# rrwick/Polypolish

Measured on AMD Instinct MI355X. Metric: assembly Mbp polished/sec at 200x coverage; bit-identical FASTA vs reference, higher is better.
Workload: dtype u8/u32 counts + f64 depth

## Files before the change

polypolish_amd/csrc/pp_k_emit.h:

```cpp
#pragma once

namespace pp {

__global__ __launch_bounds__(256) void k_sub_bases(const u8 *__restrict__ bases, const u64 *__restrict__ sub_off, u32 n_sub,
                                                   const u64 *__restrict__ src_start, u8 *__restrict__ out, u64 g_sub) {
    const u64 p0 = ((u64)blockIdx.x * blockDim.x + threadIdx.x) * 8ull;
    if (p0 >= g_sub) return;
    u32 lo = 0, hi = n_sub;
    while (hi - lo > 1) {
        const u32 mid = (lo + hi) >> 1;
        if (sub_off[mid] <= p0) lo = mid; else hi = mid;
    }
    if (p0 + 8 <= sub_off[lo + 1]) {
        u64 v;
        __builtin_memcpy(&v, bases + src_start[lo] + (p0 - sub_off[lo]), 8);
        __builtin_memcpy(out + p0, &v, 8);
        return;
    }
    for (u64 p = p0; p < min(p0 + 8, g_sub); p++) {
        while (p >= sub_off[lo + 1]) lo++;
        out[p] = bases[src_start[lo] + (p - sub_off[lo])];
    }
}

__device__ __forceinline__ u32 code_len(u8 c, u32 gp, const MultiEnt *multi, u32 n_multi) {
    if (c == 0) return 0;
    if (c < 0x80u) return 1;
    if (c != 0xFFu) return c & 0x7Fu;
    for (u32 i = 0; i < n_multi; i++)
        if (multi[i].pos == gp) return multi[i].eff;
    return 0;
}

#ifndef PP_EMIT_PPT
#define PP_EMIT_PPT 16
#endif
constexpr int EMIT_PPT = PP_EMIT_PPT;
static_assert(EMIT_PPT == 8 || EMIT_PPT == 16, "an 8- or 16-byte load of codes per thread");
constexpr int COMPACT_THREADS = TILE / EMIT_PPT;
constexpr u32 EMIT_FUSE_MAX = 4096;
template <u32 NTHREADS>
__device__ __forceinline__ u64 sum_part(const u32 *__restrict__ a, u32 n, u32 t) {
    u64 p = 0;
#pragma unroll 1
    for (u32 i0 = 4u * t; i0 < n; i0 += 16u * NTHREADS) {
        uint4 v[4];
#pragma unroll
        for (u32 j = 0; j < 4u; j++) {
            const u32 i = i0 + 4u * NTHREADS * j;
            v[j] = make_uint4(0u, 0u, 0u, 0u);
            if (i < n) v[j] = *(const uint4 *)(a + i);
        }
#pragma unroll
        for (u32 j = 0; j < 4u; j++) {
            const u32 i = i0 + 4u * NTHREADS * j;
            p += (u64)(i < n ? v[j].x : 0u) + (i + 1u < n ? v[j].y : 0u) + (i + 2u < n ? v[j].z : 0u) + (i + 3u < n ? v[j].w : 0u);
        }
    }
    return p;
}
template <u32 NTHREADS>
__device__ __forceinline__ u64 prefix_part(const u32 *__restrict__ win_coarse, const u32 *__restrict__ win_coarse2,
                                           const u32 *__restrict__ win_len, u32 w, u32 t) {
    static_assert(WIN_COARSE == 64 && WIN_COARSE2 == 64 * WIN_COARSE && NTHREADS >= 32, "two stretches of up to 64 elements: sixteen threads each");
    const u32 g = w / WIN_COARSE, g2 = w / WIN_COARSE2;
    const bool second = t >= 16u;
    const u32 *const a = second ? win_coarse + (u64)g2 * 64u : win_len + (u64)g * WIN_COARSE;
    const u32 n = second ? g - g2 * 64u : w - g * WIN_COARSE, i = 4u * (t & 15u);
    uint4 v = make_uint4(0u, 0u, 0u, 0u);
    if (t < 32u && i < n) v = *(const uint4 *)(a + i);
    u64 p = sum_part<NTHREADS>(win_coarse2, g2, t);
    if (t < 32u) p += (u64)(i < n ? v.x : 0u) + (i + 1u < n ? v.y : 0u) + (i + 2u < n ? v.z : 0u) + (i + 3u < n ? v.w : 0u);
    return p;
}

template <bool FUSED>
__device__ __forceinline__ void compact_window(u32 w, const u8 *__restrict__ code, u64 G,
                                               const u64 *__restrict__ win_out, const u32 *__restrict__ win_len, const u32 *__restrict__ win_coarse, const u32 *__restrict__ win_coarse2, u64 cap_out,
                                               const MultiEnt *__restrict__ multi,
                                               const u32 *__restrict__ counters,
                                               u8 *__restrict__ out, const u64 *__restrict__ status) {
    __shared__ u32 wsum[COMPACT_THREADS / 64];
    __shared__ u64 psum[COMPACT_THREADS / 64];
    const u32 t = threadIdx.x, lane = t & 63u, wave = t >> 6;
    const u64 p0 = (u64)w * TILE + (u64)EMIT_PPT * t;
    const bool whole = p0 + EMIT_PPT <= G;
    uint4 v = make_uint4(0u, 0u, 0u, 0u);
    if (whole) {
        if constexpr (EMIT_PPT == 16) v = *(const uint4 *)(code + p0);
        else { const uint2 h = *(const uint2 *)(code + p0); v.x = h.x; v.y = h.y; }
    }
    const u64 st = *status;
    u64 o0 = 0, o1 = 0, part = 0;
    if constexpr (FUSED) {
        o1 = win_len[w];
        part = prefix_part<COMPACT_THREADS>(win_coarse, win_coarse2, win_len, w, t);
    } else {
        o0 = win_out[w];
        o1 = win_out[w + 1];
    }
    const u32 n_multi = counters[MC_MULTI];
    asm volatile("" : "+v"(v.x), "+v"(v.y), "+v"(v.z), "+v"(v.w));
    if ((st != ~0ull) | (o1 == o0)) return;
    u8 c[EMIT_PPT];
    if (whole) {
        __builtin_memcpy(c, &v, EMIT_PPT);
    } else {
#pragma unroll
        for (int i = 0; i < EMIT_PPT; i++) c[i] = (p0 + i < G) ? code[p0 + i] : (u8)0;
    }
    u32 len[EMIT_PPT], s = 0;
    bool all_one = true;
#pragma unroll
    for (int i = 0; i < EMIT_PPT; i++) {
        len[i] = code_len(c[i], (u32)(p0 + i), multi, n_multi);
        s += len[i];
        all_one = all_one && c[i] != 0 && c[i] < 0x80u;
    }
    u32 inc = s;
    for (int o = 1; o < 64; o <<= 1) {
        u32 v2 = __shfl_up(inc, o, 64);
        if ((int)lane >= o) inc += v2;
    }
    if (lane == 63) wsum[wave] = inc;
    if constexpr (FUSED) {
        const u64 pw = wave_sum64(part);
        if (lane == 0) psum[wave] = pw;
    }
    __syncthreads();
    u32 base = 0;
    for (u32 i = 0; i < wave; i++) base += wsum[i];
    if constexpr (FUSED) {
        const u64 len_w = o1;
        o0 = 0;
        for (u32 i = 0; i < (u32)(COMPACT_THREADS / 64); i++) o0 += psum[i];
        if (o0 + len_w > cap_out) return;
    }
    u64 off = o0 + base + (inc - s);
    if (all_one) {
        __builtin_memcpy(out + off, c, EMIT_PPT);
    } else {
#pragma unroll
        for (int i = 0; i < EMIT_PPT; i++) {
            if (c[i] && c[i] < 0x80u) out[off] = c[i];
            off += len[i];
        }
    }
}

template <bool FUSED>
__device__ __forceinline__ void finalize_entries(u32 first_wave, u32 n_waves, const u8 *__restrict__ code, u64 G,
                                                 const u64 *__restrict__ win_out, u32 nwin,
                                                 const u32 *__restrict__ win_len, const u32 *__restrict__ win_coarse, const u32 *__restrict__ win_coarse2, u64 cap_out, u64 *__restrict__ total_out, u64 *status,
                                                 const MultiEnt *__restrict__ multi,
                                                 const u32 *__restrict__ counters,
                                                 const u8 *__restrict__ seq,
                                                 const u64 *__restrict__ contig_off, u32 n_contigs,
                                                 u8 *__restrict__ out, u64 *__restrict__ ctg_out) {
    const u32 n_multi = counters[MC_MULTI];
    const u32 lane = threadIdx.x & 63u;
    const u32 n_todo = n_multi + n_contigs + 1u;
    auto begin_of = [&](u32 w) -> u64 {
        if constexpr (FUSED) return wave_sum64(prefix_part<64>(win_coarse, win_coarse2, win_len, w, lane)); else return win_out[w];
    };
    for (u32 t = first_wave; t < n_todo; t += n_waves) {
        u64 gp;
        if (t < n_multi) gp = multi[t].pos; else gp = contig_off[t - n_multi];
        u64 off;
        if (gp >= G) {
            off = begin_of(nwin);
            if (FUSED && t == n_todo - 1u && lane == 0) {
                __hip_atomic_store(total_out, off, __ATOMIC_RELAXED, __HIP_MEMORY_SCOPE_AGENT);
                if (off > cap_out) report(status, off, DE_CAPACITY);
            }
        } else {
            const u32 w = (u32)(gp / TILE);
            u32 part = 0;
            bool emits;
            if constexpr (FUSED) emits = win_len[w] != 0u; else emits = win_out[w + 1] != win_out[w];
            if (emits)
                for (u64 q = (u64)w * TILE + lane; q < gp; q += 64) part += code_len(code[q], (u32)q, multi, n_multi);
            off = begin_of(w) + wave_sum(part);
        }
        if (t < n_multi) {
            if (lane == 0 && !(FUSED && off + multi[t].len > cap_out)) {
                const u8 *s = seq + multi[t].off;
                for (u32 b = 0; b < multi[t].len; b++)
                    if (s[b] != (u8)'-') out[off++] = s[b];
            }
        } else if (lane == 0) {
            __hip_atomic_store(&ctg_out[t - n_multi], off, __ATOMIC_RELAXED, __HIP_MEMORY_SCOPE_AGENT);
        }
    }
}

constexpr u32 EMIT_DONE_GROUP = 64, EMIT_DONE_STRIDE = 8;
__host__ __device__ constexpr u64 emit_done_words(u64 blocks) { return (1ull + (blocks + EMIT_DONE_GROUP - 1) / EMIT_DONE_GROUP) * EMIT_DONE_STRIDE; }
struct EmitTail {
    u64 *meta;
    u32 words;
    u32 reinit;
    u64 *host;
    u64 serial;
    u64 *done;
    u32 *zero_a, *zero_b, *zero_c, *zero_d;
    u32 n_zero;
    u32 *zero_e;
    u32 n_zero_e;
    u32 ordered;
};
__device__ __forceinline__ void emit_tail(const EmitTail &Z) {
    __shared__ u32 s_last;
    if (!Z.host) return;
#if defined(__HIP_DEVICE_COMPILE__) && !defined(__gfx950__) && !defined(__gfx942__)
#error "k_emit's last-workgroup hand-over relies on gfx942/gfx950 agent-scope store/load semantics"
#endif
    __builtin_amdgcn_s_waitcnt(0);
    __syncthreads();
    if (threadIdx.x == 0) {
        u64 *const mine = Z.done + (u64)EMIT_DONE_STRIDE * (1u + blockIdx.x / EMIT_DONE_GROUP);
        const u32 in_group = min(EMIT_DONE_GROUP, gridDim.x - blockIdx.x / EMIT_DONE_GROUP * EMIT_DONE_GROUP);
        bool last = false;
        if (__hip_atomic_fetch_add(mine, 1ull, __ATOMIC_RELAXED, __HIP_MEMORY_SCOPE_AGENT) == (u64)in_group - 1ull) {
            __hip_atomic_store(mine, 0ull, __ATOMIC_RELAXED, __HIP_MEMORY_SCOPE_AGENT);
            last = __hip_atomic_fetch_add(Z.done, 1ull, __ATOMIC_RELAXED, __HIP_MEMORY_SCOPE_AGENT) == (u64)((gridDim.x + EMIT_DONE_GROUP - 1u) / EMIT_DONE_GROUP) - 1ull;
            if (last) __hip_atomic_store(Z.done, 0ull, __ATOMIC_RELAXED, __HIP_MEMORY_SCOPE_AGENT);
        }
        s_last = last;
    }
    __syncthreads();
    if (!s_last) return;
    const u32 i0 = threadIdx.x;
    const u64 st = __hip_atomic_load(Z.meta + MW_STATUS, __ATOMIC_RELAXED, __HIP_MEMORY_SCOPE_AGENT);
    const u64 c01 = __hip_atomic_load(Z.meta + MW_COUNTERS, __ATOMIC_RELAXED, __HIP_MEMORY_SCOPE_AGENT);
    const u64 c23 = __hip_atomic_load(Z.meta + MW_COUNTERS + 1, __ATOMIC_RELAXED, __HIP_MEMORY_SCOPE_AGENT);
    u64 v = __hip_atomic_load(Z.meta + min(i0, Z.words - 1u), __ATOMIC_RELAXED, __HIP_MEMORY_SCOPE_AGENT);
    const bool flagged = (u32)c01 != 0u || (u32)c23 != 0u;
    const bool again = st == ~0ull && (Z.reinit == 2u || (Z.reinit == 1u && !flagged));
    __syncthreads();
    for (u32 i = i0; i < Z.words; i += blockDim.x) {
        if (i != i0) v = __hip_atomic_load(Z.meta + i, __ATOMIC_RELAXED, __HIP_MEMORY_SCOPE_AGENT);
        __hip_atomic_store(Z.host + i, v, __ATOMIC_RELAXED, __HIP_MEMORY_SCOPE_SYSTEM);
        if (again) Z.meta[i] = i == MW_STATUS ? ~0ull : 0ull;
    }
    if (!Z.ordered && threadIdx.x == 0) {
        __hip_atomic_store(Z.host + Z.words, again ? 1ull : 0ull, __ATOMIC_RELAXED, __HIP_MEMORY_SCOPE_SYSTEM);
        __hip_atomic_store(Z.host + Z.words + 1, Z.serial, __ATOMIC_RELAXED, __HIP_MEMORY_SCOPE_SYSTEM);
    }
    if (again) {
        for (u32 i = threadIdx.x; i < Z.n_zero_e; i += blockDim.x) Z.zero_e[i] = 0;
        if (Z.zero_a)
            for (u32 i = threadIdx.x; i < Z.n_zero; i += blockDim.x) { Z.zero_a[i] = 0; Z.zero_b[i] = 0; }
        if (Z.zero_c)
            for (u32 i = threadIdx.x; i < Z.n_zero; i += blockDim.x) { Z.zero_c[i] = 0; Z.zero_d[i] = 0; }
    }
    if (Z.ordered) {
        __builtin_amdgcn_s_waitcnt(0);
        __syncthreads();
        if (threadIdx.x == 0) {
            __hip_atomic_store(Z.host + Z.words, again ? 1ull : 0ull, __ATOMIC_RELAXED, __HIP_MEMORY_SCOPE_SYSTEM);
            __builtin_amdgcn_s_waitcnt(0);
            __hip_atomic_store(Z.host + Z.words + 1, Z.serial, __ATOMIC_RELAXED, __HIP_MEMORY_SCOPE_SYSTEM);
        }
    }
}

template <bool FUSED>
__global__ __launch_bounds__(COMPACT_THREADS) void k_emit(const u8 *__restrict__ code, u64 G, const u64 *__restrict__ win_out,
                                                          const u32 *__restrict__ win_len, const u32 *__restrict__ win_coarse, const u32 *__restrict__ win_coarse2, u64 cap_out, u64 *__restrict__ total_out,
                                                          u32 nwin, u32 n_work, const u32 *__restrict__ own_win,
                                                          const MultiEnt *__restrict__ multi,
                                                          const u32 *__restrict__ counters, const u8 *__restrict__ seq,
                                                          const u64 *__restrict__ contig_off, u32 n_contigs,
                                                          u8 *__restrict__ out, u64 *__restrict__ ctg_out,
                                                          u64 *__restrict__ status, EmitTail Z) {
    if (blockIdx.x < n_work) {
        u32 w = blockIdx.x;
        if (own_win) {
            const u32 nr = own_win[0];
            const u32 *first = own_win + 1, *before = own_win + 1 + nr;
            u32 lo = 0, hi = nr;
            while (hi - lo > 1) {
                const u32 mid = (lo + hi) >> 1;
                if (before[mid] <= w) lo = mid; else hi = mid;
            }
            w = first[lo] + (w - before[lo]);
        }
        compact_window<FUSED>(w, code, G, win_out, win_len, win_coarse, win_coarse2, cap_out, multi, counters, out, status);
    } else if (*status == ~0ull) {
        constexpr u32 WPB = COMPACT_THREADS / 64;
        finalize_entries<FUSED>((blockIdx.x - n_work) * WPB + (threadIdx.x >> 6), (gridDim.x - n_work) * WPB, code, G, win_out, nwin, win_len, win_coarse, win_coarse2, cap_out,
                         total_out, status, multi, counters, seq, contig_off, n_contigs, out, ctg_out);
    }
    emit_tail(Z);
}

}
```

Measured before the change: 18500.

## Parallelize finalize entries: vectorized prefix lengths, wave-wide sequence emit, finalize blocks first

Rewrites the finalize path of the emit kernel. Each lane now loads 16-byte chunks of the window's codes and counts emitted bytes with SWAR popcount, instead of a strided per-byte loop. The multi-entry sequence copy uses a ballot and popcount across the wave instead of a serial lane-0 loop, and the prefix computation loads speculatively without branches. Finalize blocks are reordered to the front of the grid so they start early instead of trailing the compaction blocks. This adds complexity and assumes TILE==2048.

```diff
diff --git a/polypolish_amd/csrc/pp_k_emit.h b/polypolish_amd/csrc/pp_k_emit.h
--- a/polypolish_amd/csrc/pp_k_emit.h
+++ b/polypolish_amd/csrc/pp_k_emit.h
@@ -71,6 +71,19 @@
     if (t < 32u && i < n) v = *(const uint4 *)(a + i);
     u64 p = sum_part<NTHREADS>(win_coarse2, g2, t);
     if (t < 32u) p += (u64)(i < n ? v.x : 0u) + (i + 1u < n ? v.y : 0u) + (i + 2u < n ? v.z : 0u) + (i + 3u < n ? v.w : 0u);
+    return p;
+}
+__device__ __forceinline__ u64 prefix_part_wave(const u32 *__restrict__ win_coarse, const u32 *__restrict__ win_coarse2,
+                                                const u32 *__restrict__ win_len, u32 w, u32 lane) {
+    const u32 g = w / WIN_COARSE, g2 = w / WIN_COARSE2;
+    const bool second = lane >= 16u;
+    const u32 *const a = second ? win_coarse + (u64)g2 * 64u : win_len + (u64)g * WIN_COARSE;
+    const u32 n = lane >= 32u ? 0u : (second ? g - g2 * 64u : w - g * WIN_COARSE), i = 4u * (lane & 15u);
+    const uint4 v = *(const uint4 *)(a + (i < n ? i : 0u));
+    const u32 c2 = win_coarse2[lane < g2 ? lane : 0u];
+    u64 p = (u64)(i < n ? v.x : 0u) + (i + 1u < n ? v.y : 0u) + (i + 2u < n ? v.z : 0u) + (i + 3u < n ? v.w : 0u) + (lane < g2 ? c2 : 0u);
+#pragma unroll 1
+    for (u32 j = lane + 64u; j < g2; j += 64u) p += win_coarse2[j];
     return p;
 }
 
@@ -148,6 +161,26 @@
     }
 }
 
+__device__ __forceinline__ u32 len_before(const uint4 &v, u64 q0, u64 end, const MultiEnt *multi, u32 n_multi) {
+    const u32 n = q0 < end ? (u32)min(end - q0, (u64)16) : 0u, x[4] = {v.x, v.y, v.z, v.w};
+    u32 s = 0;
+#pragma unroll
+    for (u32 j = 0; j < 4u; j++) {
+        const u32 nb = n > 4u * j ? min(n - 4u * j, 4u) : 0u;
+        const u32 y = nb == 4u ? x[j] : x[j] & ((1u << (8u * nb)) - 1u);
+        const u32 hi = y & 0x80808080u;
+        s += (u32)__popc((((y & 0x7F7F7F7Fu) + 0x7F7F7F7Fu) & 0x80808080u) & ~hi);
+        if (hi) {
+#pragma unroll 1
+            for (u32 b = 0; b < 4u; b++) {
+                const u32 c = (y >> (8u * b)) & 0xFFu;
+                if (c >= 0x80u) s += code_len((u8)c, (u32)(q0 + 4u * j + b), multi, n_multi);
+            }
+        }
+    }
+    return s;
+}
+
 template <bool FUSED>
 __device__ __forceinline__ void finalize_entries(u32 first_wave, u32 n_waves, const u8 *__restrict__ code, u64 G,
                                                  const u64 *__restrict__ win_out, u32 nwin,
@@ -161,11 +194,20 @@
     const u32 lane = threadIdx.x & 63u;
     const u32 n_todo = n_multi + n_contigs + 1u;
     auto begin_of = [&](u32 w) -> u64 {
-        if constexpr (FUSED) return wave_sum64(prefix_part<64>(win_coarse, win_coarse2, win_len, w, lane)); else return win_out[w];
+        if constexpr (FUSED) return wave_sum64(prefix_part_wave(win_coarse, win_coarse2, win_len, w, lane)); else return win_out[w];
     };
+    static_assert(TILE == 2048, "a window's codes: two 16-byte loads a lane");
     for (u32 t = first_wave; t < n_todo; t += n_waves) {
-        u64 gp;
-        if (t < n_multi) gp = multi[t].pos; else gp = contig_off[t - n_multi];
+        const bool winner = t < n_multi;
+        u64 gp, s_off = 0;
+        u32 s_len = 0;
+        if (winner) {
+            const MultiEnt m = multi[t];
+            gp = m.pos; s_off = m.off; s_len = m.len;
+        } else gp = contig_off[t - n_multi];
+        const bool has_bytes = winner && s_len != 0u;
+        u8 ch = (has_bytes ? seq + s_off : code)[has_bytes ? min(lane, s_len - 1u) : 0u];
+        if (lane >= s_len) ch = (u8)'-';
         u64 off;
         if (gp >= G) {
             off = begin_of(nwin);
@@ -175,18 +217,35 @@
             }
         } else {
             const u32 w = (u32)(gp / TILE);
+            const u64 q0 = (u64)w * TILE + 16u * lane, q1 = q0 + TILE / 2;
+            uint4 v0 = *(const uint4 *)(code + (q0 < gp ? q0 : 0)), v1 = *(const uint4 *)(code + (q1 < gp ? q1 : 0));
+            u64 o0, part64 = 0;
+            bool emits;
+            if constexpr (FUSED) {
+                emits = win_len[w] != 0u;
+                part64 = prefix_part_wave(win_coarse, win_coarse2, win_len, w, lane);
+            } else {
+                o0 = win_out[w];
+                emits = win_out[w + 1] != o0;
+            }
+            asm volatile("" : "+v"(v0.x), "+v"(v0.y), "+v"(v0.z), "+v"(v0.w), "+v"(v1.x), "+v"(v1.y), "+v"(v1.z), "+v"(v1.w), "+v"(part64));
+            if constexpr (FUSED) o0 = wave_sum64(part64);
             u32 part = 0;
-            bool emits;
-            if constexpr (FUSED) emits = win_len[w] != 0u; else emits = win_out[w + 1] != win_out[w];
             if (emits)
-                for (u64 q = (u64)w * TILE + lane; q < gp; q += 64) part += code_len(code[q], (u32)q, multi, n_multi);
-            off = begin_of(w) + wave_sum(part);
-        }
-        if (t < n_multi) {
-            if (lane == 0 && !(FUSED && off + multi[t].len > cap_out)) {
-                const u8 *s = seq + multi[t].off;
-                for (u32 b = 0; b < multi[t].len; b++)
-                    if (s[b] != (u8)'-') out[off++] = s[b];
+                part = len_before(v0, q0, gp, multi, n_multi) + len_before(v1, q1, gp, multi, n_multi);
+            off = o0 + wave_sum(part);
+        }
+        if (winner) {
+            if (!(FUSED && off + s_len > cap_out)) {
+                for (u32 b0 = 0;;) {
+                    const bool keep = ch != (u8)'-';
+                    const u64 kept = __ballot(keep);
+                    if (keep) out[off + (u32)__popcll(kept & ((1ull << lane) - 1ull))] = ch;
+                    off += (u32)__popcll(kept);
+                    b0 += 64u;
+                    if (b0 >= s_len) break;
+                    ch = b0 + lane < s_len ? seq[s_off + b0 + lane] : (u8)'-';
+                }
             }
         } else if (lane == 0) {
             __hip_atomic_store(&ctg_out[t - n_multi], off, __ATOMIC_RELAXED, __HIP_MEMORY_SCOPE_AGENT);
@@ -274,8 +333,9 @@
                                                           const u64 *__restrict__ contig_off, u32 n_contigs,
                                                           u8 *__restrict__ out, u64 *__restrict__ ctg_out,
                                                           u64 *__restrict__ status, EmitTail Z) {
-    if (blockIdx.x < n_work) {
-        u32 w = blockIdx.x;
+    const u32 n_fin = gridDim.x - n_work;
+    if (blockIdx.x >= n_fin) {
+        u32 w = blockIdx.x - n_fin;
         if (own_win) {
             const u32 nr = own_win[0];
             const u32 *first = own_win + 1, *before = own_win + 1 + nr;
@@ -289,7 +349,7 @@
         compact_window<FUSED>(w, code, G, win_out, win_len, win_coarse, win_coarse2, cap_out, multi, counters, out, status);
     } else if (*status == ~0ull) {
         constexpr u32 WPB = COMPACT_THREADS / 64;
-        finalize_entries<FUSED>((blockIdx.x - n_work) * WPB + (threadIdx.x >> 6), (gridDim.x - n_work) * WPB, code, G, win_out, nwin, win_len, win_coarse, win_coarse2, cap_out,
+        finalize_entries<FUSED>(blockIdx.x * WPB + (u32)__builtin_amdgcn_readfirstlane((int)(threadIdx.x >> 6)), n_fin * WPB, code, G, win_out, nwin, win_len, win_coarse, win_coarse2, cap_out,
                          total_out, status, multi, counters, seq, contig_off, n_contigs, out, ctg_out);
     }
     emit_tail(Z);
```

After: 18800, median of 6. No clear change (+1.6%).
